# CUAI/Edge-Proposal-Sets

Hardware: AMD Instinct MI355X
Metric: candidate edges scored/sec on ogbl-ppa (ppa-like synthetic): Adamic-Adar over the FULL 2-hop non-edge candidate set + top-4M selection (higher is better)
Workload: dtype int64

## Files before the change

edge-proposal-sets_amd/csrc/scan_pieces.hip:

```cpp
#include "eps_common.h"
#include "scan_common.h"
#include <string.h>

#define SP_EMPTY 0u
#define SP_MAXP (SP_M + 1)
#define SP_UBITS 8192
#define SP_SB 4
#define SP_PACKED_X8 8u
#define SP_MODE_RATIO 2270u
#define SP_MODE_RATIO_WIDE 8000u
#define SP_BATCH 8
#define SP_EM 128
#define SP_G 1

typedef int sp_v4i __attribute__((ext_vector_type(4)));

struct sp_params {
    const int64_t *rowptr;
    const int32_t *col;
    const int32_t *revpos;
    const uint32_t *fx32;
    const float *val;
    const float *node_w;
    float up;
// ... 68 lines not shown
    const uint32_t sv = pk_on ? p.ssum[v] - (p.heads ? (p.heads[v].y < p.ssum[v] ? p.heads[v].y : p.ssum[v]) : 0u) : 0u;
    const uint32_t smk = pk_on ? p.smax[lane <= SP_M ? lane : SP_M] : 0u;
    const int kv = __popcll(__ballot(lane >= 1 && lane < SP_M && my_bound <= v - 1));
    const int32_t hi_k = my_bound < v ? my_bound : v;
    int np = 0, k0 = 0;
    while (k0 <= kv) {
        const int32_t lo = __builtin_amdgcn_readlane(my_bound, k0);
        const uint32_t e0 = (uint32_t)__builtin_amdgcn_readlane((int)ek, k0);
        const bool in = lane > k0 && lane <= kv + 1;
        const int kd = k0 + __popcll(__ballot(in && (uint32_t)(hi_k - lo) <= direct_ids));
        const int32_t nb0 = __builtin_amdgcn_readlane(nbk, k0);
        const int kh = k0 + __popcll(__ballot(in && (ek - e0) + (uint32_t)(nbk - nb0) <= p.piece_paths));
        int kp = k0, kd16 = k0;
        uint32_t ms = 0u;
        if (pk_on) {
            const uint32_t sm0 = (uint32_t)__builtin_amdgcn_readlane((int)smk, k0);
            ms = sv < sm0 ? sv : sm0;
            const uint32_t need_s = (ms >> p.packed_dmax) + (uint32_t)dv + 2u;
            if (need_s < 0x7FFFu) kd16 = k0 + __popcll(__ballot(in && (uint32_t)(hi_k - lo) <= 2u * direct_ids));
            const uint32_t span = (uint32_t)(hi_k - lo);
            const int kb = 32 - __clz((int)((span > 2u ? span : 2u) - 1u));
            const uint32_t cap = kb >= 30 ? 0u : (1u << (31 - kb)) - 1u;
            kp = k0 + __popcll(__ballot(in && (ek - e0) + (uint32_t)(nbk - nb0) <= p.packed_paths && need_s < cap));
            if (p.wide_paths && dv <= p.wide_rows) {
                const int kw = k0 + __popcll(__ballot(in && (ek - e0) <= p.wide_paths));
                kp = kw > kp ? kw : kp;
            }
        }
        int k1;
        uint32_t flag = 0u, pq = 0u;
        const int kdd = kd16 > kd ? kd16 : kd;
        bool take_direct = kdd >= kh && kdd >= kp && kdd > k0;
        if (!take_direct && kdd > k0 && kp > kdd && kp >= kh) {
            const uint32_t pd = (uint32_t)__builtin_amdgcn_readlane((int)ek, kdd) - e0;
            const uint32_t pp = (uint32_t)__builtin_amdgcn_readlane((int)ek, kp) - e0;
            take_direct = (unsigned long long)(pp - pd) * p.mode_ratio < (unsigned long long)pd * pp;
        }
        if (take_direct && kd16 > kd) {
            k1 = kd16;
            flag = 0xC0000000u;
            uint32_t d = 0u;
            while ((ms >> d) + (uint32_t)dv + 2u >= 0x7FFFu) ++d;
            pq = d | (16u << 8);
        } else if (take_direct) {
            k1 = kd;
            flag = 0x80000000u;
        } else if (kp >= kh && kp > k0) {
            k1 = kp;
            flag = 0x40000000u;
            const uint32_t span = (uint32_t)(__builtin_amdgcn_readlane(hi_k, k1) - lo);
            const int kb = 32 - __clz((int)((span > 2u ? span : 2u) - 1u));
            if (p.wide_paths && dv <= p.wide_rows) {
                pq = (uint32_t)(kb < 31 ? kb : 31) << 8;
            } else {
                const uint32_t cap = (1u << (31 - kb)) - 1u;
                uint32_t d = 0u;
                while ((ms >> d) + (uint32_t)dv + 2u >= cap) ++d;
                pq = d | ((uint32_t)kb << 8);
            }
        } else if (kh > k0) {
            k1 = kh;
        } else {
            k1 = k0 + 1;
        }
        const uint32_t sum = (uint32_t)__builtin_amdgcn_readlane((int)ek, k1) - e0;
        if (sum) {
            emit(np, k0, k1, lo, __builtin_amdgcn_readlane(hi_k, k1), sum | flag, pq, __builtin_amdgcn_readlane(nbk, k0),
                 __builtin_amdgcn_readlane(nbk, k1));
            ++np;
        }
        k0 = k1;
    }
    return np;
}

template <int T, bool HV, bool FULL, bool PACK, bool SK = false>
__global__ __launch_bounds__(T, 4) void scan_piece_kernel(sp_params p)
{
    extern __shared__ __attribute__((aligned(16))) uint32_t lds[];
    const int slots = 1 << p.table_bits;
    uint32_t *tkey = lds;
    uint32_t *tval = lds + slots;
    uint4 *r_desc = (uint4 *)(lds + 2 * slots);
    uint32_t *ubits = lds + ((2 * slots + 4 * (T + 1) + 3) & ~3);
    uint16_t *wrank = (uint16_t *)(ubits + SP_UBITS / 32);
    __shared__ unsigned long long s_alloc;
    __shared__ int s_rbase;
    __shared__ int32_t s_pk0[SP_MAXP], s_pk1[SP_MAXP];
    __shared__ int32_t s_plo[SP_MAXP], s_phi[SP_MAXP];
    __shared__ uint32_t s_pinfo[SP_MAXP];
    __shared__ uint32_t s_pq[SP_MAXP];
    __shared__ int32_t s_pna[SP_MAXP], s_pnb[SP_MAXP];
    __shared__ int s_np;
    __shared__ unsigned int s_ticket;
    __shared__ unsigned int s_out_cur, s_out_end;
    __shared__ unsigned int s_fill_lo, s_fill_hi;
    __shared__ unsigned int s_hot;
    __shared__ uint32_t s_em[SP_EM];

    const int tid = threadIdx.x, lane = tid & 63;
    const int wib = __builtin_amdgcn_readfirstlane(tid >> 6);
    const uint32_t out_cap = p.out->capacity;
    int64_t *__restrict__ out_key = p.out->key;
    float *__restrict__ out_val = p.out->val;
    const uint32_t *__restrict__ rowptr_lo = (const uint32_t *)p.rowptr;
    const __amdgpu_buffer_rsrc_t col_rs = __builtin_amdgcn_make_buffer_rsrc((void *)p.col, 0, p.col_bytes, 0x00020000);
    const __amdgpu_buffer_rsrc_t val_rs = __builtin_amdgcn_make_buffer_rsrc((void *)(HV ? (const void *)p.val : (const void *)p.col), 0,
                                                                            p.col_bytes, 0x00020000);
    const uint32_t thr32 = sp_bar_units(p.out->threshold, p.shift);
    const uint32_t direct_ids = 2u * (uint32_t)slots;
    const bool no_bar = !FULL && thr32 <= 1u;
    const bool raw_sums = FULL || p.heads != nullptr;
    const uint32_t chunk = no_bar && direct_ids > 8192u ? direct_ids : 8192u;
    const int32_t my_bound = p.bounds[lane <= SP_M ? lane : SP_M];

    for (int i = tid; i < 2 * slots; i += T) lds[i] = 0u;
    for (int i = tid; i < SP_UBITS / 32; i += T) ubits[i] = 0u;
    for (int i = tid; i < SP_EM; i += T) s_em[i] = 0u;
    if (tid == 0) {
        s_out_cur = 0u;
        s_out_end = 0u;
        s_fill_lo = 0u;
        s_fill_hi = 0u;
        s_alloc = 0ull;
    }
    bool sketch_seen = false;
    unsigned long long n_cand = 0;
    uint32_t new_keys = 0u;
    const unsigned int ncol = (unsigned int)p.n_columns;
    const unsigned int batch_from = p.batch_from;
    auto first_of = [&](unsigned int tk) { return tk < batch_from ? tk : batch_from + (tk - batch_from) * SP_BATCH; };
    unsigned int t = blockIdx.x < batch_from ? blockIdx.x : first_of(blockIdx.x);
    unsigned int t_end = t + (blockIdx.x < batch_from ? 1u : SP_BATCH);
    sp_barrier();

    while (t < ncol) {
        const bool last_of_ticket = t + 1u >= t_end || t + 1u >= ncol;
        unsigned int t_next = 0;
        if (tid == 0 && last_of_ticket) t_next = gridDim.x + atomicAdd(p.next_col, 1u);
        int32_t v, dv;
        uint32_t vb;
        uint4 cra = make_uint4(0u, 0u, 0u, 0u), crb = make_uint4(0u, 0u, 0u, 0u);
        if (FULL || p.colrec) {
            cra = p.colrec[2 * (size_t)t];
            crb = p.colrec[2 * (size_t)t + 1];
            v = (int32_t)cra.x;
            vb = cra.y;
            dv = (int32_t)cra.z;
        } else {
            v = p.columns[t];
            vb = rowptr_lo[2 * (size_t)v];
            dv = (int32_t)(rowptr_lo[2 * (size_t)v + 2] - vb);
        }
        const int32_t *__restrict__ vcol = p.col + vb;
        const int32_t *__restrict__ vrev = p.revpos + vb;
        const int rounds = (dv + T - 1) / T;
        const bool single = rounds == 1;
        uint32_t xv = 0u, thr_v = thr32;
        bool bad_head = false;
        if (FULL || p.heads) {
            const uint2 hd = (FULL || p.colrec) ? make_uint2(cra.w, crb.x) : p.heads[v];
            xv = hd.x;
            if (thr32 < SP_FLAG) {
                bad_head = hd.y >= thr32;
                thr_v = thr32 - hd.y;
            }
            if (bad_head && tid == 0) atomicOr(p.status, 4u);
            if ((FULL || p.ssum) && thr32 < SP_FLAG && ((FULL || p.colrec) ? crb.y : p.ssum[v]) < thr32) bad_head = true;
        }
        if (dv > 0 && v > 0 && !bad_head) {
            uint32_t my_w = 0, my_rev = 0, my_base = 0, my_fx = 0;
            uint32_t cut_first = 0u;
            if (PACK && single && tid < dv) {
                const uint4 pa = p.pack[2 * ((size_t)vb + (size_t)tid)];
                my_w = pa.x;
                my_base = pa.y;
                my_fx = pa.z;
                my_rev = pa.w & 0xFFFFu;
                cut_first = pa.w >> 16;
            }
            if (!PACK && single && tid < dv) {
                my_w = (uint32_t)vcol[tid];
                my_rev = (uint32_t)vrev[tid];
            }
            if (!PACK && single && tid < dv) {
                my_base = (FULL || p.rowrec) ? p.rowrec[(size_t)my_w * 32 + 16] : rowptr_lo[2 * (size_t)my_w];
                my_fx = HV ? __builtin_bit_cast(uint32_t, (p.val[vb + tid] * p.node_w[my_w]) * p.up)
                           : ((FULL || p.rowrec) ? p.rowrec[(size_t)my_w * 32 + 17] : p.fx32[my_w]);
            }
            if (!FULL && wib == 0 && !p.plan) {
                const uint32_t pwk = lane < SP_M ? p.wpaths[(size_t)v * SP_M + lane] : 0u;
                const int32_t nbk = lane >= 1 && lane <= SP_M ? (int32_t)p.cuts[(size_t)v * SP_M + lane - 1] : 0;
                const int np = sp_plan_column(p, v, dv, lane, my_bound, pwk, nbk, direct_ids,
                                              [&](int i, int k0, int k1, int32_t lo, int32_t hi, uint32_t info, uint32_t pq, int32_t na, int32_t nb) {
                                                  if (lane == 0) {
                                                      s_pk0[i] = k0;
                                                      s_pk1[i] = k1;
                                                      s_plo[i] = lo;
                                                      s_phi[i] = hi;
                                                      s_pinfo[i] = info;
                                                      s_pq[i] = pq;
                                                      s_pna[i] = na;
                                                      s_pnb[i] = nb;
                                                  }
                                              });
                if (lane == 0) s_np = np;
            } else if (FULL || p.plan) {
                const uint32_t pb = (FULL || p.colrec) ? crb.z : p.pptr[v];
                const int np = (FULL || p.colrec) ? (int)crb.w : (int)(p.pptr[v + 1] - pb);
                if (tid < np) {
                    const uint4 rec = p.plan[pb + (uint32_t)tid];
                    const int k1 = (int)((rec.y >> 8) & 0xFFu);
                    const int32_t bk = p.bounds[k1];
                    s_pinfo[tid] = rec.x;
                    s_pk0[tid] = (int)(rec.y & 0xFFu);
                    s_pk1[tid] = k1;
                    s_pq[tid] = rec.y >> 16;
                    s_pna[tid] = (int32_t)(rec.z & 0xFFFFu);
                    s_pnb[tid] = (int32_t)(rec.z >> 16);
                    s_plo[tid] = (int32_t)rec.w;
                    s_phi[tid] = bk < v ? bk : v;
                }
                if (tid == 0) s_np = np;
            }
            sp_barrier();
            const int np = s_np;
            uint32_t cut_ahead = 0u, seg_from = 0u;
            const uint16_t *__restrict__ cut_tab = (FULL || p.rowrec) ? (const uint16_t *)p.rowrec : p.cuts;
            const size_t cut_ld = (FULL || p.rowrec) ? 64u : (size_t)SP_M;
            const uint16_t *__restrict__ pack16 = (const uint16_t *)p.pack;
            if (PACK) cut_ahead = cut_first;
            else if (single && tid < dv && np > 0) cut_ahead = cut_tab[(size_t)my_w * cut_ld + s_pk1[0] - 1];

            for (int pi = 0; pi < np; ++pi) {
                const int k0 = s_pk0[pi], k1 = s_pk1[pi];
                const int na = s_pna[pi], nb = s_pnb[pi];
                const uint32_t info = s_pinfo[pi];
                const bool direct = (info >> 31) != 0u;
                const bool d16 = !HV && (info >> 30) == 3u;
                const bool packed_kind = !HV && (info >> 30) == 1u;
                const bool sketch = SK && packed_kind && single && p.sketch != 0u && thr_v < SP_FLAG;
                const bool packed = packed_kind && !sketch;
                const bool quant = packed || d16;
                const uint32_t ppaths = info & 0x3FFFFFFFu;
                const uint32_t pq = quant ? s_pq[pi] : 0u;
                const uint32_t pk_d = pq & 0xFFu, pk_sb = quant ? 32u - (pq >> 8) : 16u;
                const uint32_t pk_flag = quant ? 1u << (pk_sb - 1u) : 0u;
                const uint32_t pk_thr = thr_v >= SP_FLAG ? 0xFFFFFFFFu : ((thr_v >> pk_d) ? (thr_v >> pk_d) : 1u);
                const int32_t lo_id = s_plo[pi], hi_id = s_phi[pi];
                const uint32_t pkeys = ppaths + (uint32_t)(nb - na);
                int plog = 0;
                if (!direct && !packed && !sketch && pkeys > p.piece_paths) {
                    const uint32_t q = (pkeys + p.piece_paths - 1u) / p.piece_paths;
                    plog = 32 - __clz((int)(q - 1u)) + 1;
                }
                const uint32_t parts = 1u << plog;
                int bits;
                {
                    const uint32_t per = (pkeys + parts - 1u) >> plog;
                    const int max_bits = packed || sketch ? p.table_bits + 1 : p.table_bits;
                    const int want = per > 1u ? 33 - __clz((int)(per - 1u)) : 1;
                    bits = want < 10 ? 10 : (want > max_bits ? max_bits : want);
                }
                const uint32_t mask = (1u << bits) - 1u;
                const uint32_t span = (uint32_t)(hi_id - lo_id);
                const uint32_t scan_slots = d16 ? (span + 1u) >> 1 : direct ? span : (1u << bits);
                const uint32_t cand_max = direct ? span : (1u << bits);
                if (tid == 0) {
                    s_hot = 0u;
                    uint32_t need = ppaths < cand_max ? ppaths : cand_max;
                    if (!no_bar && need > 1024u) need = 1024u;
                    if (need > chunk) need = chunk;
                    const uint32_t left = s_out_cur < s_out_end ? s_out_end - s_out_cur : 0u;
                    if (left < need) {
                        s_fill_lo = s_out_cur < out_cap ? s_out_cur : out_cap;
                        s_fill_hi = left ? (s_out_end < out_cap ? s_out_end : out_cap) : s_fill_lo;
                        const unsigned long long b64 = atomicAdd(&p.out->count, (unsigned long long)chunk);
                        const uint32_t b = b64 < (unsigned long long)out_cap ? (uint32_t)b64 : out_cap;
                        s_out_cur = b;
                        s_out_end = b + chunk;
                    }
                }
                uint32_t seg_a = 0u, seg_len = 0u;
                if (single && tid < dv) {
                    const uint32_t b = cut_ahead < my_rev ? cut_ahead : my_rev;
                    seg_a = seg_from;
                    seg_len = (uint32_t)tid < xv ? 0u : b - seg_from;
                    seg_from = b;
                    if (pi + 1 < np)
                        cut_ahead = PACK && pi + 1 <= 8 ? pack16[((size_t)vb + (size_t)tid) * 16 + 7 + (pi + 1)]
                                                        : cut_tab[(size_t)my_w * cut_ld + s_pk1[pi + 1] - 1];
                }
                auto emit = [&](uint32_t u, uint32_t sum) {
                    uint32_t pos = atomicAdd(&s_out_cur, 1u);
                    if (pos >= s_out_end) {
                        const unsigned long long q = atomicAdd(&p.out->count, 1ull);
                        pos = q < (unsigned long long)out_cap ? (uint32_t)q : out_cap;
                    }
                    if (pos < out_cap) {
                        out_key[pos] = ((int64_t)v << 32) | (int64_t)u;
                        out_val[pos] = raw_sums ? __builtin_bit_cast(float, sum) : (float)sum * p.scale;
                    }
                };
                for (uint32_t part = 0; part < parts; ++part) {
                    for (int j = sketch ? nb : single ? tid : na + tid; j < nb; j += T) {
                        const uint32_t u = single ? my_w : (uint32_t)vcol[j];
                        if (j >= na && (int32_t)u >= lo_id && (int32_t)u < hi_id) {
                            if (d16) {
                                const uint32_t o = u - (uint32_t)lo_id;
                                atomicOr(&lds[o >> 1], 0x8000u << ((o & 1u) << 4));
                            } else if (direct) {
                                lds[u - (uint32_t)lo_id] = SP_FLAG;
                            } else if (packed) {
                                const uint32_t mix = sp_mix(u);
                                uint32_t h = mix >> (32 - bits);
                                const uint32_t st = ((mix >> 7) | 1u) & mask;
                                const uint32_t word = ((u - (uint32_t)lo_id) << pk_sb) | pk_flag;
                                for (uint32_t tries = 0; tries <= mask; ++tries) {
                                    if (atomicCAS(&lds[h], 0u, word) == 0u) break;
                                    h = (h + st) & mask;
                                }
                            } else {
                                const uint32_t mix = sp_mix(u);
                                if ((mix & (parts - 1u)) == part) {
                                    uint32_t h = mix >> (32 - bits);
                                    const uint32_t st = ((mix >> 7) | 1u) & mask;
                                    for (uint32_t tries = 0; tries <= mask; ++tries) {
                                        if (atomicCAS(&tkey[h], SP_EMPTY, u + 1u) == SP_EMPTY) {
                                            tval[h] = SP_FLAG;
                                            break;
                                        }
                                        h = (h + st) & mask;
                                    }
                                }
                            }
                        }
                    }
                    for (int r = 0; r < rounds; ++r) {
                        const int j = r * T + tid;
                        uint32_t w = my_w, rev = my_rev, base = my_base, fx = my_fx;
                        uint32_t len = 0u, a = 0u;
                        if (single) {
                            a = seg_a;
                            len = seg_len;
                        } else if (j < dv) {
                            w = (uint32_t)vcol[j];
                            rev = (uint32_t)vrev[j];
                            base = (FULL || p.rowrec) ? p.rowrec[(size_t)w * 32 + 16] : rowptr_lo[2 * (size_t)w];
                            fx = HV ? __builtin_bit_cast(uint32_t, (p.val[vb + j] * p.node_w[w]) * p.up)
                                    : ((FULL || p.rowrec) ? p.rowrec[(size_t)w * 32 + 17] : p.fx32[w]);
                            const uint16_t *crow = cut_tab + (size_t)w * cut_ld;
                            uint32_t b = crow[k1 - 1];
                            if (k0 > 0) a = crow[k0 - 1];
                            a = a < rev ? a : rev;
                            b = b < rev ? b : rev;
                            len = (uint32_t)j < xv ? 0u : b - a;
                        }
                        const int units = (int)((len + 3u) >> 2);
                        const int flag = units > 0 ? 1 : 0;
                        const int incl_c = sp_wave_incl_scan(units | (flag << 24));
                        const int incl = incl_c & 0xFFFFFF, incl_f = (int)((uint32_t)incl_c >> 24);
                        unsigned long long got = 0ull;
                        if (lane == 63) got = atomicAdd(&s_alloc, ((unsigned long long)(uint32_t)incl << 32) | (unsigned long long)(uint32_t)incl_f);
                        const int woff = __builtin_amdgcn_readlane((int)(got >> 32), 63);
                        const int woff_f = __builtin_amdgcn_readlane((int)(uint32_t)got, 63);
                        const uint32_t a_u = (uint32_t)(incl - units + woff);
                        if (flag) {
                            const int d = incl_f - 1 + woff_f;
                            r_desc[d] = make_uint4(base + a, len, quant ? (fx + ((1u << pk_d) - 1u)) >> pk_d : fx, a_u);
                            if (a_u < (uint32_t)SP_UBITS) atomicOr(&ubits[a_u >> 5], 1u << (a_u & 31u));
                        }
                        sp_barrier();
                        if (s_fill_hi > s_fill_lo) {
                            const uint32_t f0 = s_fill_lo, f1 = s_fill_hi;
                            for (uint32_t i = f0 + (uint32_t)tid; i < f1; i += T) {
                                out_key[i] = -1;
                                out_val[i] = -__builtin_inff();
                            }
                        }
                        const int total = (int)(s_alloc >> 32);
                        for (uint32_t ulo = 0; ulo < (uint32_t)total; ulo += SP_UBITS) {
                            const uint32_t uhi = ulo + SP_UBITS < (uint32_t)total ? ulo + SP_UBITS : (uint32_t)total;
                            if (ulo > 0u) {
                                for (int i = tid; i < SP_UBITS / 32; i += T) ubits[i] = 0u;
                                if (tid == 0) s_rbase = 0;
                                sp_barrier();
                                const unsigned long long before = __ballot(flag && a_u + (uint32_t)units <= ulo);
                                if (lane == 0 && before) atomicAdd(&s_rbase, __popcll(before));
                                if (flag && a_u + (uint32_t)units > ulo && a_u < uhi) {
                                    const uint32_t pos = (a_u > ulo ? a_u : ulo) - ulo;
                                    atomicOr(&ubits[pos >> 5], 1u << (pos & 31));
                                }
                                sp_barrier();
                            }
                            const int rbase = ulo > 0u ? s_rbase : 0;
                            {
                                const uint4 b4 = *(const uint4 *)(ubits + 4 * lane);
                                const int c0 = __popc(b4.x), c1 = c0 + __popc(b4.y), c2 = c1 + __popc(b4.z), c3 = c2 + __popc(b4.w);
                                const int ex = sp_wave_incl_scan(c3) - c3;
                                uint2 pk;
                                pk.x = (uint32_t)ex | ((uint32_t)(ex + c0) << 16);
                                pk.y = (uint32_t)(ex + c1) | ((uint32_t)(ex + c2) << 16);
                                *(uint2 *)(wrank + 4 * lane) = pk;
                                asm volatile("s_waitcnt lgkmcnt(0)" ::: "memory");
                            }
                        auto fetch_group = [&](int it0, sp_unit (&f)[SP_G]) {
                            int lo[SP_G];
#pragma unroll
                            for (int q = 0; q < SP_G; ++q) {
                                const uint32_t sr = (uint32_t)((it0 + q) * T + tid);
                                const uint32_t wd = sr < SP_UBITS ? sr >> 5 : 0u;
                                const uint32_t bits = ubits[wd];
                                const int rk = (int)wrank[wd];
                                lo[q] = rbase + rk + __popc(bits & ((2u << (sr & 31u)) - 1u)) - 1;
                                lo[q] = lo[q] < 0 ? 0 : lo[q];
                            }
#pragma unroll
                            for (int q = 0; q < SP_G; ++q) {
                                const int s = (int)ulo + (it0 + q) * T + tid;
                                const uint4 rd = r_desc[lo[q]];
                                const uint32_t us = rd.w, rl = rd.y, rs = rd.x;
                                f[q].fx = rd.z;
                                const bool in = s < (int)uhi;
                                const int off = (s - (int)us) * 4;
                                int left = (int)rl - off;
                                left = in ? left : 0;
                                f[q].nvalid = left < 0 ? 0 : (left > 4 ? 4 : left);
                                const uint32_t at = in ? rs + (uint32_t)off : (p.col_bytes >> 2);
                                f[q].u4 = __builtin_amdgcn_raw_buffer_load_b128(col_rs, (int)(at * 4u), 0, 0);
                                if (HV) f[q].a4 = __builtin_bit_cast(sp_v4f, __builtin_amdgcn_raw_buffer_load_b128(val_rs, (int)(at * 4u), 0, 0));
                            }
                        };
                        auto path_fx = [&](const sp_unit &f, int e) -> uint32_t {
                            if (!HV) return f.fx;
                            return (uint32_t)__builtin_ceilf(f.a4[e] * __builtin_bit_cast(float, f.fx)) + 1u;
                        };
                        auto consume_group = [&](const sp_unit (&f)[SP_G]) {
                            if (sketch) {
                                const uint32_t half = 1u << (bits - 1);
#pragma unroll
                                for (int q = 0; q < SP_G; ++q)
#pragma unroll
                                    for (int e = 0; e < 4; ++e)
                                        if (e < f[q].nvalid) {
                                            const uint32_t id = (uint32_t)f[q].u4[e];
                                            atomicAdd(&lds[sp_mix(id) >> (33 - bits)], f[q].fx);
                                            atomicAdd(&lds[half + (sp_mix2(id) >> (33 - bits))], f[q].fx);
                                        }
                            } else if (d16) {
#pragma unroll
                                for (int q = 0; q < SP_G; ++q)
#pragma unroll
                                    for (int e = 0; e < 4; ++e)
                                        if (e < f[q].nvalid) {
                                            const uint32_t o = (uint32_t)(f[q].u4[e] - lo_id);
                                            atomicAdd(&lds[o >> 1], f[q].fx << ((o & 1u) << 4));
                                        }
                            } else if (direct) {
#pragma unroll
                                for (int q = 0; q < SP_G; ++q)
#pragma unroll
                                    for (int e = 0; e < 4; ++e)
                                        if (e < f[q].nvalid) atomicAdd(&lds[(uint32_t)(f[q].u4[e] - lo_id)], path_fx(f[q], e));
// ... 141 lines not shown
                            const int n_iter = (int)(uhi - ulo + T - 1) / T;
                            sp_unit fa[SP_G], fb[SP_G];
                            fetch_group(0, fa);
                            if (n_iter <= SP_G) {
                                consume_group(fa);
                            } else {
                                for (int it0 = 0; it0 < n_iter; it0 += 2 * SP_G) {
                                    fetch_group(it0 + SP_G, fb);
                                    consume_group(fa);
                                    fetch_group(it0 + 2 * SP_G, fa);
                                    consume_group(fb);
                                }
                            }
                        }
                        if (sketch) {
                            if (tid == 0 && !sketch_seen) atomicOr(p.status, 16u);
                            sketch_seen = true;
                            sp_barrier();
                            const uint32_t half = 1u << (bits - 1);
                            {
                                uint32_t mx = 0u;
                                for (uint32_t i = 4u * (uint32_t)tid; i < half; i += 4u * T) {
                                    const uint4 a4 = *(const uint4 *)(lds + i);
                                    const uint32_t m01 = a4.x > a4.y ? a4.x : a4.y, m23 = a4.z > a4.w ? a4.z : a4.w;
                                    const uint32_t m = m01 > m23 ? m01 : m23;
                                    mx = m > mx ? m : mx;
                                }
                                if (__ballot(mx >= thr_v) && lane == 0) s_hot = 1u;
                            }
                            sp_barrier();
                            if (s_hot) {
                            const int n_iter = (int)(uhi - ulo + T - 1) / T;
                            auto report = [&](uint32_t u, uint32_t est) {
                                int a = na, b = nb;
                                while (a < b) {
                                    const int mid = (a + b) >> 1;
                                    if (vcol[mid] < (int32_t)u) a = mid + 1; else b = mid;
                                }
                                if (a < nb && vcol[a] == (int32_t)u) return;
                                const uint32_t em_mask = (p.sketch >> 1 ? p.sketch >> 1 : (uint32_t)SP_EM) - 1u;
                                uint32_t h = (sp_mix(u) >> 9) & em_mask;
                                for (uint32_t tries = 0; tries <= em_mask; ++tries) {
                                    const uint32_t old = atomicCAS(&s_em[h], 0u, u + 1u);
                                    if (old == 0u) {
                                        emit(u, est);
                                        return;
                                    }
                                    if (old == u + 1u) return;
                                    h = (h + 1u) & em_mask;
                                }
                                atomicOr(p.status, 8u);
                            };
                            auto look = [&](const sp_unit (&f)[SP_G]) {
                                uint32_t est[4 * SP_G];
#pragma unroll
                                for (int i = 0; i < 4 * SP_G; ++i) {
                                    const uint32_t id = (uint32_t)f[i >> 2].u4[i & 3];
                                    const uint32_t ea = lds[sp_mix(id) >> (33 - bits)], eb = lds[half + (sp_mix2(id) >> (33 - bits))];
                                    est[i] = ea < eb ? ea : eb;
                                }
#pragma unroll
                                for (int i = 0; i < 4 * SP_G; ++i)
                                    if ((i & 3) < f[i >> 2].nvalid && est[i] >= thr_v) report((uint32_t)f[i >> 2].u4[i & 3], est[i]);
                            };
                            sp_unit fa[SP_G], fb[SP_G];
                            fetch_group(0, fa);
                            if (n_iter <= SP_G) {
                                look(fa);
                            } else {
                                for (int it0 = 0; it0 < n_iter; it0 += 2 * SP_G) {
                                    fetch_group(it0 + SP_G, fb);
                                    look(fa);
                                    fetch_group(it0 + 2 * SP_G, fa);
                                    look(fb);
                                }
                            }
                            }
                        }
                            if (uhi < (uint32_t)total) sp_barrier();
                        }
                        sp_barrier();
                        for (int i = tid; i < SP_UBITS / 32; i += T) ubits[i] = 0u;
                        if (tid == 0) {
                            s_alloc = 0ull;
                            s_fill_hi = 0u;
                        }
                        if (r + 1 < rounds) sp_barrier();
                    }
                    uint32_t cnt_here = 0u;
                    const int thr_s = thr_v >= SP_FLAG ? 0x7FFFFFFF : (int)thr_v;
                    if (d16) {
                        const int thr_h = pk_thr >= 0x8000u ? 0x7FFFFFFF : (int)(pk_thr << 16);
                        const uint32_t n4 = (scan_slots + 3u) & ~3u;
                        for (uint32_t i0 = 0; i0 < n4; i0 += 4u * SP_SB * T) {
                            uint4 s4[SP_SB];
#pragma unroll
                            for (int b = 0; b < SP_SB; ++b) {
                                const uint32_t i = i0 + 4u * T * b + 4u * tid;
                                s4[b] = i < n4 ? *(const uint4 *)(lds + i) : make_uint4(0u, 0u, 0u, 0u);
                            }
#pragma unroll
                            for (int b = 0; b < SP_SB; ++b) {
                                const uint32_t i = i0 + 4u * T * b + 4u * tid;
                                if (i < n4) *(uint4 *)(lds + i) = make_uint4(0u, 0u, 0u, 0u);
                                const uint32_t wv[4] = {s4[b].x, s4[b].y, s4[b].z, s4[b].w};
                                int x[8];
#pragma unroll
                                for (int e = 0; e < 4; ++e) {
                                    x[2 * e] = (int)(wv[e] << 16);
                                    x[2 * e + 1] = (int)(wv[e] & 0xFFFF0000u);
                                }
#pragma unroll
                                for (int e = 0; e < 8; ++e) cnt_here += x[e] > 0 ? 1u : 0u;
                                int m = x[0];
#pragma unroll
                                for (int e = 1; e < 8; ++e) m = x[e] > m ? x[e] : m;
                                if (m >= thr_h) {
#pragma unroll
                                    for (int e = 0; e < 8; ++e)
                                        if (x[e] >= thr_h) emit((uint32_t)lo_id + 2u * i + e, ((uint32_t)x[e] >> 16) << pk_d);
                                }
                            }
                        }
                    } else if (direct) {
                        const uint32_t n4 = (scan_slots + 3u) & ~3u;
                        for (uint32_t i0 = 0; i0 < n4; i0 += 4u * SP_SB * T) {
                            uint4 s4[SP_SB];
#pragma unroll
                            for (int b = 0; b < SP_SB; ++b) {
                                const uint32_t i = i0 + 4u * T * b + 4u * tid;
                                s4[b] = i < n4 ? *(const uint4 *)(lds + i) : make_uint4(0u, 0u, 0u, 0u);
                            }
#pragma unroll
                            for (int b = 0; b < SP_SB; ++b) {
                                const uint32_t i = i0 + 4u * T * b + 4u * tid;
                                if (i < n4) *(uint4 *)(lds + i) = make_uint4(0u, 0u, 0u, 0u);
                                const int sv[4] = {(int)s4[b].x, (int)s4[b].y, (int)s4[b].z, (int)s4[b].w};
#pragma unroll
                                for (int e = 0; e < 4; ++e) cnt_here += sv[e] > 0 ? 1u : 0u;
                                const int m01 = sv[0] > sv[1] ? sv[0] : sv[1], m23 = sv[2] > sv[3] ? sv[2] : sv[3];
                                if ((m01 > m23 ? m01 : m23) >= thr_s) {
#pragma unroll
                                    for (int e = 0; e < 4; ++e)
                                        if (sv[e] >= thr_s) emit((uint32_t)lo_id + i + e, (uint32_t)sv[e]);
                                }
                            }
                        }
                    } else if (sketch) {
                        for (uint32_t i = 4u * (uint32_t)tid; i < scan_slots; i += 4u * T) *(uint4 *)(lds + i) = make_uint4(0u, 0u, 0u, 0u);
                        for (int i = tid; i < SP_EM; i += T) s_em[i] = 0u;
                    } else if (packed) {
                        const uint32_t kb = 32u - pk_sb;
                        const int thr_p = pk_thr >= pk_flag ? 0x7FFFFFFF : (int)(pk_thr << kb);
                        for (uint32_t i0 = 0; i0 < scan_slots; i0 += 4u * SP_SB * T) {
                            uint4 s4[SP_SB];
#pragma unroll
                            for (int b = 0; b < SP_SB; ++b) {
                                const uint32_t i = i0 + 4u * T * b + 4u * tid;
                                s4[b] = i < scan_slots ? *(const uint4 *)(lds + i) : make_uint4(0u, 0u, 0u, 0u);
                            }
#pragma unroll
                            for (int b = 0; b < SP_SB; ++b) {
                                const uint32_t i = i0 + 4u * T * b + 4u * tid;
                                if (i < scan_slots) *(uint4 *)(lds + i) = make_uint4(0u, 0u, 0u, 0u);
                                const uint32_t sv[4] = {s4[b].x, s4[b].y, s4[b].z, s4[b].w};
                                const int x[4] = {(int)(sv[0] << kb), (int)(sv[1] << kb), (int)(sv[2] << kb), (int)(sv[3] << kb)};
                                const int m01 = x[0] > x[1] ? x[0] : x[1], m23 = x[2] > x[3] ? x[2] : x[3];
                                if ((m01 > m23 ? m01 : m23) >= thr_p) {
#pragma unroll
                                    for (int e = 0; e < 4; ++e)
                                        if (x[e] >= thr_p) emit((uint32_t)lo_id + (sv[e] >> pk_sb), ((uint32_t)x[e] >> kb) << pk_d);
                                }
                            }
                        }
                    } else {
                        for (uint32_t i0 = 0; i0 < scan_slots; i0 += 4u * SP_SB * T) {
                            uint4 s4[SP_SB];
#pragma unroll
                            for (int b = 0; b < SP_SB; ++b) {
                                const uint32_t i = i0 + 4u * T * b + 4u * tid;
                                s4[b] = i < scan_slots ? *(const uint4 *)(tval + i) : make_uint4(0u, 0u, 0u, 0u);
                            }
#pragma unroll
                            for (int b = 0; b < SP_SB; ++b) {
                                const uint32_t i = i0 + 4u * T * b + 4u * tid;
                                const int sv[4] = {(int)s4[b].x, (int)s4[b].y, (int)s4[b].z, (int)s4[b].w};
                                const int m01 = sv[0] > sv[1] ? sv[0] : sv[1], m23 = sv[2] > sv[3] ? sv[2] : sv[3];
                                if ((m01 > m23 ? m01 : m23) >= thr_s) {
#pragma unroll
                                    for (int e = 0; e < 4; ++e)
                                        if (sv[e] >= thr_s) emit(tkey[i + e] - 1u, (uint32_t)sv[e]);
                                }
                                if (i < scan_slots) {
                                    *(uint4 *)(tkey + i) = make_uint4(0u, 0u, 0u, 0u);
                                    *(uint4 *)(tval + i) = make_uint4(0u, 0u, 0u, 0u);
                                }
                            }
                        }
                    }
                    n_cand += (unsigned long long)cnt_here + (unsigned long long)new_keys;
                    new_keys = 0u;
                    sp_barrier();
                }
            }
        }
        if (!last_of_ticket) {
            ++t;
            sp_barrier();
            continue;
        }
        if (tid == 0) s_ticket = t_next;
        sp_barrier();
        const unsigned int tk = s_ticket;
        sp_barrier();
        t = first_of(tk);
        t_end = t + (tk < batch_from ? 1u : SP_BATCH);
    }
    {
        const uint32_t f0 = s_out_cur < out_cap ? s_out_cur : out_cap, f1 = s_out_end < out_cap ? s_out_end : out_cap;
        for (uint32_t i = f0 + (uint32_t)tid; i < f1; i += T) {
            out_key[i] = -1;
            out_val[i] = -__builtin_inff();
        }
    }
    {
        unsigned long long x = n_cand;
#pragma unroll
        for (int d = 32; d >= 1; d >>= 1) x += __shfl_xor(x, d);
        if (lane == 0 && x) atomicAdd(&p.out->n_candidates, x);
    }
}

__global__ void sp_cuts_kernel(const int64_t *__restrict__ rowptr, const int32_t *__restrict__ col, int64_t n_nodes,
                               const int32_t *__restrict__ bounds, uint16_t *__restrict__ cuts)
{
    const int64_t stride = (int64_t)gridDim.x * blockDim.x;
    for (int64_t i = (int64_t)blockIdx.x * blockDim.x + threadIdx.x; i < n_nodes * SP_M; i += stride) {
        const int64_t w = i / SP_M;
        const int k = (int)(i % SP_M);
        const int32_t bound = bounds[k + 1];
        int64_t lo = rowptr[w], hi = rowptr[w + 1];
        const int64_t wb = lo;
        while (lo < hi) {
            const int64_t mid = (lo + hi) >> 1;
            if (col[mid] < bound) lo = mid + 1; else hi = mid;
        }
        cuts[i] = (uint16_t)(lo - wb);
    }
}

__global__ void sp_window_paths_kernel(const int64_t *__restrict__ rowptr, const int32_t *__restrict__ col,
                                       const int32_t *__restrict__ revpos, const uint16_t *__restrict__ cuts, int64_t n_nodes,
                                       const uint2 *__restrict__ heads, uint32_t *__restrict__ wpaths,
                                       const int32_t *__restrict__ columns, int64_t n_columns)
{
    const int lane = threadIdx.x & 63;
    const int64_t wave = ((int64_t)blockIdx.x * blockDim.x + threadIdx.x) >> 6;
    const int64_t n_waves = ((int64_t)gridDim.x * blockDim.x) >> 6;
    const int64_t count = columns ? n_columns : n_nodes;
    for (int64_t idx = wave; idx < count; idx += n_waves) {
        const int64_t v = columns ? (int64_t)columns[idx] : idx;
        const int64_t b = rowptr[v] + (heads ? (int64_t)heads[v].x : 0ll), e = rowptr[v + 1];
        uint32_t cnt[SP_M];
#pragma unroll
        for (int k = 0; k < SP_M; ++k) cnt[k] = 0u;
        for (int64_t i = b + lane; i < e; i += 64) {
            const uint32_t rev = (uint32_t)revpos[i];
            const uint4 *row = (const uint4 *)(cuts + (size_t)col[i] * SP_M);
            uint32_t prev = 0u;
#pragma unroll
            for (int q = 0; q < SP_M / 8; ++q) {
                const uint4 c = row[q];
                const uint32_t wds[4] = {c.x, c.y, c.z, c.w};
#pragma unroll
                for (int h = 0; h < 4; ++h) {
                    uint32_t a = wds[h] & 0xFFFFu, bb = wds[h] >> 16;
                    a = a < rev ? a : rev;
                    bb = bb < rev ? bb : rev;
                    cnt[q * 8 + h * 2] += a - prev;
                    cnt[q * 8 + h * 2 + 1] += bb - a;
                    prev = bb;
                }
            }
        }
        uint32_t mine = 0u;
// ... 688 lines not shown
    }
    if ((threadIdx.x & 63) == 0) {
        if (re) atomicAdd(&out[0], re);
        if (all) atomicAdd(&out[1], all);
    }
}

extern "C" int eps_scan_plan_rewalk(const uint32_t *plan, int64_t n_rec, int32_t variant, unsigned long long *out2, void *stream)
{
    EPS_REQUIRE(n_rec >= 0 && out2 && variant >= 0 && variant <= 2, "eps_scan_plan_rewalk: bad argument");
    hipStream_t s = (hipStream_t)stream;
    if (hipMemsetAsync(out2, 0, 2 * sizeof(unsigned long long), s) != hipSuccess) {
        eps_set_error("eps_scan_plan_rewalk: cannot clear the result");
        return EPS_ELAUNCH;
    }
    if (n_rec == 0) return EPS_OK;
    EPS_REQUIRE(plan && ((uintptr_t)plan & 15) == 0, "eps_scan_plan_rewalk: plan must be 16-byte aligned");
    int64_t blocks = (n_rec + 255) / 256;
    if (blocks > 2048) blocks = 2048;
    hipLaunchKernelGGL(sp_rewalk_kernel, dim3((unsigned)blocks), dim3(256), 0, s, (const uint4 *)plan, n_rec,
                       (1u << sp_bits_of[variant]) / 2u, out2);
    EPS_CHECK_LAUNCH("eps_scan_plan_rewalk");
    return EPS_OK;
}

static int sp_launch(const int64_t *rowptr, const int32_t *col, const float *val, const int32_t *revpos, const uint32_t *fx32,
                     const float *node_w, const uint16_t *cuts, const uint32_t *wpaths, const uint32_t *ssum, const uint32_t *smax,
                     const uint32_t *pptr, const uint32_t *plan, const uint32_t *heads, const uint32_t *rowrec, const uint32_t *pack,
                     const int32_t *bounds, int64_t n_nodes, int64_t nnz, const int32_t *columns, const uint32_t *colrec, int64_t n_columns, int64_t batch_from,
                     int32_t shift, int32_t variant, eps_survivors *out, uint32_t *status, void *stream)
{
    EPS_REQUIRE(n_nodes >= 0 && n_columns >= 0 && nnz >= 0, "eps_scan_screen: negative size");
    EPS_REQUIRE(status, "eps_scan_screen: null pointer");
    hipStream_t s = (hipStream_t)stream;
    if (hipMemsetAsync(status, 0, sizeof(uint32_t), s) != hipSuccess) {
        eps_set_error("eps_scan_screen: cannot clear the status word");
        return EPS_ELAUNCH;
    }
    if (n_columns == 0 || n_nodes == 0) return EPS_OK;
    EPS_REQUIRE(rowptr && col && revpos && cuts && wpaths && bounds && columns && out, "eps_scan_screen: null pointer");
    EPS_REQUIRE(nnz < (1ll << 30), "eps_scan_screen: col[] is addressed with 32-bit byte offsets (nnz < 2^30)");
    EPS_REQUIRE(n_nodes < (1ll << 31) && n_columns < (1ll << 31), "eps_scan_screen: too many nodes / columns");
    const uint32_t sketch_arg = (uint32_t)SP_VARIANT_SKETCH(variant);
    EPS_REQUIRE(!SP_VARIANT_WIDE(variant) || ((sketch_arg & 1u) && plan && !val && SP_VARIANT_GEOM(variant) == 2),
                "eps_scan_screen: a plan with wide packed pieces (variant bit 24) is for sketch launches (bit 16) of the 256-thread geometry");
    const int32_t dmax_arg = SP_VARIANT_DMAX(variant);
    variant = SP_VARIANT_GEOM(variant);
    EPS_REQUIRE(shift >= 0 && shift <= 40 && variant >= 0 && variant <= 2, "eps_scan_screen: bad shift / variant");
    EPS_REQUIRE(((uintptr_t)cuts & 15) == 0, "eps_scan_screen: cuts must be 16-byte aligned");
    EPS_REQUIRE(((uintptr_t)colrec & 15) == 0 && ((uintptr_t)rowrec & 127) == 0, "eps_scan_screen: misaligned column / row records");
    EPS_REQUIRE(!colrec || plan, "eps_scan_screen: column records come with the plan table they were built from");
    EPS_REQUIRE((pptr == nullptr) == (plan == nullptr) && ((uintptr_t)plan & 15) == 0, "eps_scan_screen: pptr and plan come together, 16-byte aligned");
    const int T = sp_threads_of[variant], bits = sp_bits_of[variant];
    unsigned int *counter = nullptr;
    const int rc = eps_take_counter(&counter, s, "eps_scan_screen");
    if (rc) return rc;
    sp_params p;
    memset(&p, 0, sizeof p);
    p.rowptr = rowptr;
    p.col = col;
    p.revpos = revpos;
    p.fx32 = fx32;
    p.val = val;
    p.node_w = node_w;
    p.up = ldexpf(1.0f, shift) * (1.0f + ldexpf(1.0f, -20));
    sp_plan_geometry(p, cuts, wpaths, ssum, smax, bounds, n_nodes, shift, variant, dmax_arg);
    p.pptr = pptr;
    p.plan = (const uint4 *)plan;
    p.heads = (const uint2 *)heads;
    p.rowrec = rowrec;
    p.pack = (const uint4 *)pack;
    p.colrec = (const uint4 *)colrec;
    p.columns = columns;
    p.n_columns = (int32_t)n_columns;
    p.batch_from = batch_from < 0 || batch_from > n_columns ? (uint32_t)n_columns : (uint32_t)batch_from;
    p.sketch = val || !(sketch_arg & 1u) ? 0u : sketch_arg;
    p.col_bytes = (uint32_t)(nnz * 4);
    p.scale = ldexpf(1.0f, -shift);
    p.next_col = counter;
    p.out = out;
    p.status = status;
    int64_t blocks = (int64_t)eps_num_cus() * sp_per_cu[variant];
    if (blocks > n_columns) blocks = n_columns;
    const size_t lds = ((size_t)(2 << bits) + 4 * (size_t)(T + 1) + 8) * 4 + (SP_UBITS / 32) * 6 + 32;
    void (*kern)(sp_params) =
        val ? (variant == 0 ? scan_piece_kernel<512, true, false, false> : variant == 1 ? scan_piece_kernel<1024, true, false, false>
                                                                                       : scan_piece_kernel<256, true, false, false>)
            : (variant == 0 ? scan_piece_kernel<512, false, false, false> : variant == 1 ? scan_piece_kernel<1024, false, false, false>
                                                                                         : scan_piece_kernel<256, false, false, false>);
    const bool full = !val && variant == 2 && plan && colrec && rowrec && heads && ssum;
    EPS_REQUIRE(!pack || full, "eps_scan_screen: the column pack serves the main launch only (variant 2, plan, records, heads, sum bounds)");
    if (full) kern = pack ? scan_piece_kernel<256, false, true, true> : scan_piece_kernel<256, false, true, false>;
    if (p.sketch && variant == 2)
        kern = full ? (pack ? scan_piece_kernel<256, false, true, true, true> : scan_piece_kernel<256, false, true, false, true>)
                    : scan_piece_kernel<256, false, false, false, true>;
    else
        p.sketch = 0u;
    if (hipFuncSetAttribute((const void *)kern, hipFuncAttributeMaxDynamicSharedMemorySize, (int)lds) != hipSuccess) {
        eps_set_error("eps_scan_screen: cannot reserve %zu bytes of LDS", lds);
        return EPS_ELAUNCH;
    }
    hipLaunchKernelGGL(kern, dim3((unsigned)blocks), dim3(T), lds, s, p);
    EPS_CHECK_LAUNCH("eps_scan_screen");
    return EPS_OK;
}

__global__ void scan_pieces_warm_kernel() {}
extern "C" void eps_warm_scan_pieces(void *stream) { hipLaunchKernelGGL(scan_pieces_warm_kernel, dim3(1), dim3(1), 0, (hipStream_t)stream); }
```

Measured before the change: 1282 billion.

## Double-buffer segment descriptors to prefetch next piece in sketch kernel

In the sketch (SK) kernel variant, the scan now keeps two sets of unit bitmaps and allocation counters and builds the next piece's segment descriptors at the end of the current piece, which lets it skip a block barrier and describe step on the following piece. Known-edge marking can be deferred until after the barrier, so the direct-table write becomes an atomicOr. The output fill of sentinel values moves from all threads after a barrier to wave 0. Per-piece plan fields are packed into fewer shared arrays. The cost is extra LDS and more complex control flow, and only the sketch path changes.

Result: slower. 1256 billion (-2.0%).

```diff
diff --git a/edge-proposal-sets_amd/csrc/scan_pieces.hip b/edge-proposal-sets_amd/csrc/scan_pieces.hip
--- a/edge-proposal-sets_amd/csrc/scan_pieces.hip
+++ b/edge-proposal-sets_amd/csrc/scan_pieces.hip
@@ -174,15 +174,15 @@
     uint32_t *tkey = lds;
     uint32_t *tval = lds + slots;
     uint4 *r_desc = (uint4 *)(lds + 2 * slots);
-    uint32_t *ubits = lds + ((2 * slots + 4 * (T + 1) + 3) & ~3);
-    uint16_t *wrank = (uint16_t *)(ubits + SP_UBITS / 32);
-    __shared__ unsigned long long s_alloc;
+    constexpr bool RO = SK;
+    uint32_t *ubits2 = lds + ((2 * slots + 4 * (T + 1) + 3) & ~3);
+    uint16_t *wrank = (uint16_t *)(ubits2 + (RO ? 2 : 1) * (SP_UBITS / 32));
+    __shared__ unsigned long long s_alloc2[RO ? 2 : 1];
     __shared__ int s_rbase;
-    __shared__ int32_t s_pk0[SP_MAXP], s_pk1[SP_MAXP];
+    __shared__ uint32_t s_pky[SP_MAXP];
     __shared__ int32_t s_plo[SP_MAXP], s_phi[SP_MAXP];
     __shared__ uint32_t s_pinfo[SP_MAXP];
-    __shared__ uint32_t s_pq[SP_MAXP];
-    __shared__ int32_t s_pna[SP_MAXP], s_pnb[SP_MAXP];
+    __shared__ uint32_t s_pnab[SP_MAXP];
     __shared__ int s_np;
     __shared__ unsigned int s_ticket;
     __shared__ unsigned int s_out_cur, s_out_end;
@@ -207,15 +207,17 @@
     const int32_t my_bound = p.bounds[lane <= SP_M ? lane : SP_M];
 
     for (int i = tid; i < 2 * slots; i += T) lds[i] = 0u;
-    for (int i = tid; i < SP_UBITS / 32; i += T) ubits[i] = 0u;
+    for (int i = tid; i < (RO ? 2 : 1) * (SP_UBITS / 32); i += T) ubits2[i] = 0u;
     for (int i = tid; i < SP_EM; i += T) s_em[i] = 0u;
     if (tid == 0) {
         s_out_cur = 0u;
         s_out_end = 0u;
         s_fill_lo = 0u;
         s_fill_hi = 0u;
-        s_alloc = 0ull;
-    }
+        s_alloc2[0] = 0ull;
+        if (RO) s_alloc2[RO ? 1 : 0] = 0ull;
+    }
+    int cur = 0;
     bool sketch_seen = false;
     unsigned long long n_cand = 0;
     uint32_t new_keys = 0u;
@@ -286,14 +288,11 @@
                 const int np = sp_plan_column(p, v, dv, lane, my_bound, pwk, nbk, direct_ids,
                                               [&](int i, int k0, int k1, int32_t lo, int32_t hi, uint32_t info, uint32_t pq, int32_t na, int32_t nb) {
                                                   if (lane == 0) {
-                                                      s_pk0[i] = k0;
-                                                      s_pk1[i] = k1;
+                                                      s_pky[i] = (uint32_t)k0 | ((uint32_t)k1 << 8) | (pq << 16);
                                                       s_plo[i] = lo;
                                                       s_phi[i] = hi;
                                                       s_pinfo[i] = info;
-                                                      s_pq[i] = pq;
-                                                      s_pna[i] = na;
-                                                      s_pnb[i] = nb;
+                                                      s_pnab[i] = (uint32_t)na | ((uint32_t)nb << 16);
                                                   }
                                               });
                 if (lane == 0) s_np = np;
@@ -305,11 +304,8 @@
                     const int k1 = (int)((rec.y >> 8) & 0xFFu);
                     const int32_t bk = p.bounds[k1];
                     s_pinfo[tid] = rec.x;
-                    s_pk0[tid] = (int)(rec.y & 0xFFu);
-                    s_pk1[tid] = k1;
-                    s_pq[tid] = rec.y >> 16;
-                    s_pna[tid] = (int32_t)(rec.z & 0xFFFFu);
-                    s_pnb[tid] = (int32_t)(rec.z >> 16);
+                    s_pky[tid] = rec.y;
+                    s_pnab[tid] = rec.z;
                     s_plo[tid] = (int32_t)rec.w;
                     s_phi[tid] = bk < v ? bk : v;
                 }
@@ -322,11 +318,13 @@
             const size_t cut_ld = (FULL || p.rowrec) ? 64u : (size_t)SP_M;
             const uint16_t *__restrict__ pack16 = (const uint16_t *)p.pack;
             if (PACK) cut_ahead = cut_first;
-            else if (single && tid < dv && np > 0) cut_ahead = cut_tab[(size_t)my_w * cut_ld + s_pk1[0] - 1];
-
+            else if (single && tid < dv && np > 0) cut_ahead = cut_tab[(size_t)my_w * cut_ld + ((s_pky[0] >> 8) & 0xFFu) - 1];
+
+            bool pre = false;
             for (int pi = 0; pi < np; ++pi) {
-                const int k0 = s_pk0[pi], k1 = s_pk1[pi];
-                const int na = s_pna[pi], nb = s_pnb[pi];
+                const uint32_t pky = s_pky[pi], pnab = s_pnab[pi];
+                const int k0 = (int)(pky & 0xFFu), k1 = (int)((pky >> 8) & 0xFFu);
+                const int na = (int)(pnab & 0xFFFFu), nb = (int)(pnab >> 16);
                 const uint32_t info = s_pinfo[pi];
                 const bool direct = (info >> 31) != 0u;
                 const bool d16 = !HV && (info >> 30) == 3u;
@@ -335,7 +333,7 @@
                 const bool packed = packed_kind && !sketch;
                 const bool quant = packed || d16;
                 const uint32_t ppaths = info & 0x3FFFFFFFu;
-                const uint32_t pq = quant ? s_pq[pi] : 0u;
+                const uint32_t pq = quant ? pky >> 16 : 0u;
                 const uint32_t pk_d = pq & 0xFFu, pk_sb = quant ? 32u - (pq >> 8) : 16u;
                 const uint32_t pk_flag = quant ? 1u << (pk_sb - 1u) : 0u;
                 const uint32_t pk_thr = thr_v >= SP_FLAG ? 0xFFFFFFFFu : ((thr_v >> pk_d) ? (thr_v >> pk_d) : 1u);
@@ -358,30 +356,76 @@
                 const uint32_t span = (uint32_t)(hi_id - lo_id);
                 const uint32_t scan_slots = d16 ? (span + 1u) >> 1 : direct ? span : (1u << bits);
                 const uint32_t cand_max = direct ? span : (1u << bits);
-                if (tid == 0) {
-                    s_hot = 0u;
-                    uint32_t need = ppaths < cand_max ? ppaths : cand_max;
-                    if (!no_bar && need > 1024u) need = 1024u;
-                    if (need > chunk) need = chunk;
-                    const uint32_t left = s_out_cur < s_out_end ? s_out_end - s_out_cur : 0u;
-                    if (left < need) {
-                        s_fill_lo = s_out_cur < out_cap ? s_out_cur : out_cap;
-                        s_fill_hi = left ? (s_out_end < out_cap ? s_out_end : out_cap) : s_fill_lo;
-                        const unsigned long long b64 = atomicAdd(&p.out->count, (unsigned long long)chunk);
-                        const uint32_t b = b64 < (unsigned long long)out_cap ? (uint32_t)b64 : out_cap;
-                        s_out_cur = b;
-                        s_out_end = b + chunk;
+                if (RO ? wib == 0 : tid == 0) {
+                    uint32_t f0 = 0u, f1 = 0u;
+                    if (tid == 0) {
+                        s_hot = 0u;
+                        uint32_t need = ppaths < cand_max ? ppaths : cand_max;
+                        if (!no_bar && need > 1024u) need = 1024u;
+                        if (need > chunk) need = chunk;
+                        const uint32_t left = s_out_cur < s_out_end ? s_out_end - s_out_cur : 0u;
+                        if (left < need) {
+                            f0 = s_out_cur < out_cap ? s_out_cur : out_cap;
+                            f1 = left ? (s_out_end < out_cap ? s_out_end : out_cap) : f0;
+                            const unsigned long long b64 = atomicAdd(&p.out->count, (unsigned long long)chunk);
+                            const uint32_t b = b64 < (unsigned long long)out_cap ? (uint32_t)b64 : out_cap;
+                            s_out_cur = b;
+                            s_out_end = b + chunk;
+                            if (!RO) {
+                                s_fill_lo = f0;
+                                s_fill_hi = f1;
+                            }
+                        }
+                    }
+                    if (RO) {
+                        f0 = (uint32_t)__builtin_amdgcn_readfirstlane((int)f0);
+                        f1 = (uint32_t)__builtin_amdgcn_readfirstlane((int)f1);
+                        for (uint32_t i = f0 + (uint32_t)lane; i < f1; i += 64u) {
+                            out_key[i] = -1;
+                            out_val[i] = -__builtin_inff();
+                        }
                     }
                 }
                 uint32_t seg_a = 0u, seg_len = 0u;
-                if (single && tid < dv) {
-                    const uint32_t b = cut_ahead < my_rev ? cut_ahead : my_rev;
-                    seg_a = seg_from;
-                    seg_len = (uint32_t)tid < xv ? 0u : b - seg_from;
-                    seg_from = b;
-                    if (pi + 1 < np)
-                        cut_ahead = PACK && pi + 1 <= 8 ? pack16[((size_t)vb + (size_t)tid) * 16 + 7 + (pi + 1)]
-                                                        : cut_tab[(size_t)my_w * cut_ld + s_pk1[pi + 1] - 1];
+                auto take_segment = [&](int q) {
+                    if (single && tid < dv) {
+                        const uint32_t b = cut_ahead < my_rev ? cut_ahead : my_rev;
+                        seg_a = seg_from;
+                        seg_len = (uint32_t)tid < xv ? 0u : b - seg_from;
+                        seg_from = b;
+                        if (q + 1 < np)
+                            cut_ahead = PACK && q + 1 <= 8 ? pack16[((size_t)vb + (size_t)tid) * 16 + 7 + (q + 1)]
+                                                           : cut_tab[(size_t)my_w * cut_ld + ((s_pky[q + 1] >> 8) & 0xFFu) - 1];
+                    }
+                };
+                if (!(RO && pre)) take_segment(pi);
+                auto describe = [&](uint32_t seg0, uint32_t len, uint32_t fxq, int buf, uint32_t &a_u, int &units, int &flag) {
+                    units = (int)((len + 3u) >> 2);
+                    flag = units > 0 ? 1 : 0;
+                    const int incl_c = sp_wave_incl_scan(units | (flag << 24));
+                    const int incl = incl_c & 0xFFFFFF, incl_f = (int)((uint32_t)incl_c >> 24);
+                    unsigned long long got = 0ull;
+                    if (lane == 63) got = atomicAdd(&s_alloc2[buf], ((unsigned long long)(uint32_t)incl << 32) | (unsigned long long)(uint32_t)incl_f);
+                    const int woff = __builtin_amdgcn_readlane((int)(got >> 32), 63);
+                    const int woff_f = __builtin_amdgcn_readlane((int)(uint32_t)got, 63);
+                    a_u = (uint32_t)(incl - units + woff);
+                    if (flag) {
+                        const int d = incl_f - 1 + woff_f;
+                        r_desc[d] = make_uint4(seg0, len, fxq, a_u);
+                        if (a_u < (uint32_t)SP_UBITS) atomicOr(&ubits2[buf * (SP_UBITS / 32) + (a_u >> 5)], 1u << (a_u & 31u));
+                    }
+                };
+                const bool ke_late = RO && single && parts == 1u && (direct || sketch);
+                bool pre_next = false;
+                uint32_t nx_d = 0u;
+                if (RO && single && pi + 1 < np) {
+                    const uint32_t ninfo = s_pinfo[pi + 1], nnab = s_pnab[pi + 1];
+                    const bool n_direct = (ninfo >> 31) != 0u, n_pk = (ninfo >> 30) == 1u;
+                    const bool n_sketch = n_pk && p.sketch != 0u && thr_v < SP_FLAG;
+                    const uint32_t nkeys = (ninfo & 0x3FFFFFFFu) + ((nnab >> 16) - (nnab & 0xFFFFu));
+                    pre_next = (n_direct || n_pk || nkeys <= p.piece_paths) && ((ninfo & 0x3FFFFFFFu) >> 2) + (uint32_t)dv <= (uint32_t)SP_UBITS;
+                    const bool n_quant = (n_pk && !n_sketch) || (ninfo >> 30) == 3u;
+                    nx_d = n_quant ? (s_pky[pi + 1] >> 16) & 0xFFu : 0u;
                 }
                 auto emit = [&](uint32_t u, uint32_t sum) {
                     uint32_t pos = atomicAdd(&s_out_cur, 1u);
@@ -395,6 +439,7 @@
                     }
                 };
                 for (uint32_t part = 0; part < parts; ++part) {
+                    auto known_edges = [&]() {
                     for (int j = sketch ? nb : single ? tid : na + tid; j < nb; j += T) {
                         const uint32_t u = single ? my_w : (uint32_t)vcol[j];
                         if (j >= na && (int32_t)u >= lo_id && (int32_t)u < hi_id) {
@@ -402,7 +447,7 @@
                                 const uint32_t o = u - (uint32_t)lo_id;
                                 atomicOr(&lds[o >> 1], 0x8000u << ((o & 1u) << 4));
                             } else if (direct) {
-                                lds[u - (uint32_t)lo_id] = SP_FLAG;
+                                atomicOr(&lds[u - (uint32_t)lo_id], SP_FLAG);
                             } else if (packed) {
                                 const uint32_t mix = sp_mix(u);
                                 uint32_t h = mix >> (32 - bits);
@@ -428,6 +473,8 @@
                             }
                         }
                     }
+                    };
+                    if (!ke_late) known_edges();
                     for (int r = 0; r < rounds; ++r) {
                         const int j = r * T + tid;
                         uint32_t w = my_w, rev = my_rev, base = my_base, fx = my_fx;
@@ -448,29 +495,20 @@
                             b = b < rev ? b : rev;
                             len = (uint32_t)j < xv ? 0u : b - a;
                         }
-                        const int units = (int)((len + 3u) >> 2);
-                        const int flag = units > 0 ? 1 : 0;
-                        const int incl_c = sp_wave_incl_scan(units | (flag << 24));
-                        const int incl = incl_c & 0xFFFFFF, incl_f = (int)((uint32_t)incl_c >> 24);
-                        unsigned long long got = 0ull;
-                        if (lane == 63) got = atomicAdd(&s_alloc, ((unsigned long long)(uint32_t)incl << 32) | (unsigned long long)(uint32_t)incl_f);
-                        const int woff = __builtin_amdgcn_readlane((int)(got >> 32), 63);
-                        const int woff_f = __builtin_amdgcn_readlane((int)(uint32_t)got, 63);
-                        const uint32_t a_u = (uint32_t)(incl - units + woff);
-                        if (flag) {
-                            const int d = incl_f - 1 + woff_f;
-                            r_desc[d] = make_uint4(base + a, len, quant ? (fx + ((1u << pk_d) - 1u)) >> pk_d : fx, a_u);
-                            if (a_u < (uint32_t)SP_UBITS) atomicOr(&ubits[a_u >> 5], 1u << (a_u & 31u));
-                        }
-                        sp_barrier();
-                        if (s_fill_hi > s_fill_lo) {
+                        uint32_t a_u = 0u;
+                        int units = 0, flag = 0;
+                        if (!(RO && pre)) describe(base + a, len, quant ? (fx + ((1u << pk_d) - 1u)) >> pk_d : fx, cur, a_u, units, flag);
+                        if (!(RO && pre) || !ke_late) sp_barrier();
+                        if (ke_late) known_edges();
+                        uint32_t *ubits = ubits2 + cur * (SP_UBITS / 32);
+                        if (!RO && s_fill_hi > s_fill_lo) {
                             const uint32_t f0 = s_fill_lo, f1 = s_fill_hi;
                             for (uint32_t i = f0 + (uint32_t)tid; i < f1; i += T) {
                                 out_key[i] = -1;
                                 out_val[i] = -__builtin_inff();
                             }
                         }
-                        const int total = (int)(s_alloc >> 32);
+                        const int total = (int)(s_alloc2[cur] >> 32);
                         for (uint32_t ulo = 0; ulo < (uint32_t)total; ulo += SP_UBITS) {
                             const uint32_t uhi = ulo + SP_UBITS < (uint32_t)total ? ulo + SP_UBITS : (uint32_t)total;
                             if (ulo > 0u) {
@@ -778,10 +816,16 @@
                         sp_barrier();
                         for (int i = tid; i < SP_UBITS / 32; i += T) ubits[i] = 0u;
                         if (tid == 0) {
-                            s_alloc = 0ull;
-                            s_fill_hi = 0u;
+                            s_alloc2[cur] = 0ull;
+                            if (!RO) s_fill_hi = 0u;
                         }
                         if (r + 1 < rounds) sp_barrier();
+                    }
+                    if (RO && pre_next && part + 1u == parts) {
+                        take_segment(pi + 1);
+                        uint32_t a_u;
+                        int units, flag;
+                        describe(my_base + seg_a, seg_len, (my_fx + ((1u << nx_d) - 1u)) >> nx_d, cur ^ 1, a_u, units, flag);
                     }
                     uint32_t cnt_here = 0u;
                     const int thr_s = thr_v >= SP_FLAG ? 0x7FFFFFFF : (int)thr_v;
@@ -897,6 +941,10 @@
                     n_cand += (unsigned long long)cnt_here + (unsigned long long)new_keys;
                     new_keys = 0u;
                     sp_barrier();
+                }
+                if (RO) {
+                    pre = pre_next;
+                    cur ^= pre ? 1 : 0;
                 }
             }
         }
@@ -1751,7 +1799,7 @@
     p.status = status;
     int64_t blocks = (int64_t)eps_num_cus() * sp_per_cu[variant];
     if (blocks > n_columns) blocks = n_columns;
-    const size_t lds = ((size_t)(2 << bits) + 4 * (size_t)(T + 1) + 8) * 4 + (SP_UBITS / 32) * 6 + 32;
+    size_t lds = ((size_t)(2 << bits) + 4 * (size_t)(T + 1) + 8) * 4 + (SP_UBITS / 32) * 6 + 32;
     void (*kern)(sp_params) =
         val ? (variant == 0 ? scan_piece_kernel<512, true, false, false> : variant == 1 ? scan_piece_kernel<1024, true, false, false>
                                                                                        : scan_piece_kernel<256, true, false, false>)
@@ -1760,11 +1808,13 @@
     const bool full = !val && variant == 2 && plan && colrec && rowrec && heads && ssum;
     EPS_REQUIRE(!pack || full, "eps_scan_screen: the column pack serves the main launch only (variant 2, plan, records, heads, sum bounds)");
     if (full) kern = pack ? scan_piece_kernel<256, false, true, true> : scan_piece_kernel<256, false, true, false>;
-    if (p.sketch && variant == 2)
+    if (p.sketch && variant == 2) {
+        lds += (SP_UBITS / 32) * 4;
         kern = full ? (pack ? scan_piece_kernel<256, false, true, true, true> : scan_piece_kernel<256, false, true, false, true>)
                     : scan_piece_kernel<256, false, false, false, true>;
-    else
+    } else {
         p.sketch = 0u;
+    }
     if (hipFuncSetAttribute((const void *)kern, hipFuncAttributeMaxDynamicSharedMemorySize, (int)lds) != hipSuccess) {
         eps_set_error("eps_scan_screen: cannot reserve %zu bytes of LDS", lds);
         return EPS_ELAUNCH;
```
